# homopolymer/RAMBL

Measured on AMD Instinct MI355X. Metric: reads/sec into POA (150bp, ~1.5k-node graph), higher is better.
Workload: dtype f64

## Files before the change

rambl_amd/csrc/sc_api.cpp:

```cpp
#include <malloc.h>

#include <cmath>

#include "sc_ctx.hpp"

using namespace sc;
struct sc_ctx { Ctx c; sc_ctx(int device, const CtxPlan& plan) : c(device, plan) {} };

extern "C" {

int sc_host_plan(int stream_count, int local_world, double cpus, int* out) {
    if (!out || stream_count < 1) return SC_ERR_ARG;
    host_plan(stream_count, local_world > 0 ? local_world : local_world_size(), cpus > 0 ? cpus : cpu_budget_host(), out);
    return SC_OK;
}

int sc_ctx_create(int device, int stream_count, sc_ctx** out) {
    if (!out) return SC_ERR_ARG;
    *out = nullptr;
    setenv("GPU_MAX_HW_QUEUES", "16", 0);
    int ndev = 0;
    if (hipGetDeviceCount(&ndev) != hipSuccess || ndev <= 0 || device < 0 || device >= ndev) return SC_ERR_NO_DEVICE;
    hipDeviceProp_t prop;
    if (hipGetDeviceProperties(&prop, device) != hipSuccess) return SC_ERR_NO_DEVICE;
// ... 266 lines not shown
            f.labels[(size_t)e] = (uint8_t)(r >= 0 ? ent_sym[r] : 0);
        }
        for (int r = 0, q = 0; r < n_ent; r++) { f.ent_cn[(size_t)(e0 + r)] = ent_cn[r]; qoff[(size_t)(e0 + r)] = q; q += ent_cn[r]; }
        const hipStream_t st = w.st;
        const std::vector<int> mptr(mate_off, mate_off + n_reads + 1), midx(mate_idx, mate_idx + nm);
        JobDev jd = w.job_dev(w.passthrough, f, qoff, mptr, midx, n_reads, std::max<long>(Q, 1), n_ent, Q * n_sweeps);
        auto slot = [](int s) { return (s * 37 + 5) % MAXS; };
        std::vector<double> rows((size_t)jd.ll_stride * MAXS, 0.0);
        for (int s = 0; s < S; s++) std::memcpy(&rows[(size_t)slot(s) * jd.ll_stride], ll + (size_t)s * n_reads, sizeof(double) * n_reads);
        jd.ll = upload(w.passthrough, w.b_ll, rows, st);
        std::vector<uint8_t> hv(has, has + n_reads);
        hv.resize((size_t)n_reads + 8, 0);
        jd.has = upload(w.passthrough, w.b_has, hv, st);
        std::vector<double> u(U, U + Q * n_sweeps);
        u.resize((size_t)(Q * n_sweeps + 2048), 0.5);
        std::vector<float> uf(u.begin(), u.end());
        DevBuf b_u, b_uf;
        jd.U = upload(w.passthrough, b_u, u, st);
        jd.Uf = upload(w.passthrough, b_uf, uf, st);
        const JobDev* jd_dev = (const JobDev*)w.b_jobdev.ensure(sizeof(JobBlock));
        HIPCHK(hipMemcpyAsync((void*)jd_dev, &jd, sizeof jd, hipMemcpyHostToDevice, st));

        LevelParams& P = *w.Ph;
        for (int s = 0; s < S; s++) P.sp[s] = StrainParam{slot(s), E, 1, 0, a0[s], 0.0};
        LevelHdr H{};
        H.mode = MODE_SAMPLE; H.S = S; H.e0 = e0; H.e1 = E; H.Q = (int)Q; H.n_sweeps = n_sweeps;
        H.n_copy = 0; H.do_update = 0; H.seq = 1;
        std::memset(w.Rh, 0, sizeof(LevelResult));
        const LevelItem it = w.level_item(jd_dev, H, KMAX);
        const int kind = item_kind(it.kind);
        const int done = launch_level(st, it, n_reads);
        HIPCHK(hipGetLastError());
        HIPCHK(hipStreamSynchronize(st));
        const LevelResult& R = *w.Rh;
        if (R.seq != 1u || R.error) throw ScError(SC_ERR_INTERNAL, "the sampler level did not complete");
        for (int s = 0; s < S; s++) kdraw[s] = R.kdraw[s];
        std::memcpy(cnt, R.cnt, sizeof(unsigned) * (size_t)S * KMAX);
        out[0] = (long)R.n_draws; out[1] = (long)R.n_slow; out[2] = (long)R.n_exact; out[3] = (long)R.n_pass; out[4] = kind; out[5] = done;
        return SC_OK;
    } catch (const ScError& ex) { std::lock_guard<std::mutex> lk(ctx->mu); ctx->last_error = ex.what(); return ex.code; }
    catch (const std::exception& ex) { std::lock_guard<std::mutex> lk(ctx->mu); ctx->last_error = ex.what(); return SC_ERR_HIP; }
}
int sc_roi_release(sc_ctx* h, int handle) {
    if (!h) return SC_ERR_ARG;
    std::lock_guard<std::mutex> lk(h->c.mu);
    auto it = h->c.jobs.find(handle);
    if (it == h->c.jobs.end() || it->second->status != 1) return SC_ERR_ARG;
    h->c.jobs.erase(it);
    return SC_OK;
}

int sc_msa_align(sc_ctx* h, const char* seq_text, const int* seq_off, int n, char* rows_out, long cap, int* ncol_out) {
    if (!h || !seq_text || !seq_off || n < 1 || !ncol_out) return SC_ERR_ARG;
    Ctx* ctx = &h->c;
// ... 19 lines not shown
```

rambl_amd/csrc/sc_ctx.hpp:

```cpp
#pragma once
#include <atomic>
#include <condition_variable>
#include <deque>
#include <map>
#include <memory>
#include <mutex>
#include <thread>

#include "../../include/straincall_hip.h"
#include "sc_device.hpp"
#include "sc_fiber.hpp"
#include "sc_graph.hpp"
#include "sc_host.hpp"
#include "sc_plan.hpp"

namespace sc {

void launch_edge_support(hipStream_t st, const int* out_ptr, const int* out_node, const int* pool_ptr, const int* pool_rid,
                         const int* pool_cn, const uint8_t* node_is_end, const int* edge_src, int n_edges, int sorted,
                         int* support);
void launch_msa(hipStream_t st, const MsaDev& d);
void launch_thread(hipStream_t st, const ThreadDev& d, int* pool_sorted);
int init_graph_kernels();
bool level_wants_grid(int n_reads, const LevelHdr& h);
int launch_level_grid(hipStream_t st, const JobDev* job, int n_reads, const LevelHdr& h, int kind, const LevelParams* P, LevelResult* R, bool lone);
int launch_level(hipStream_t st, const LevelItem& it, int n_reads);
int level_kind(const LevelHdr& h);
int level_lds_kb(const LevelHdr& h, int K);
int level_table_capacity();
void launch_level_batch(hipStream_t st, int kind, const LevelBatch& b, int n);
void launch_level_any(hipStream_t st, const LevelBatch& b, int n);
void launch_resident(hipStream_t st, const ResidentArgs& a, int slots);
int init_level_kernels();
inline int init_kernels() { return init_level_kernels() | init_graph_kernels(); }

struct Job {
    int handle = 0;
    std::string ref;
    std::vector<AlignedRead> reads;
    std::vector<int> mate_off, mate_idx;
    sc_params params{};
    std::vector<std::string> seqs;
    std::vector<double> abund;
    std::string graph_dump, trace;
    std::vector<int> edge_support;
    std::vector<int> thr_count, thr_first, thr_pool;
    std::vector<int> thr_smin, thr_emin, thr_tmin;
    std::string thr_sym;
    sc_stats stats{};
// ... 118 lines not shown
};

struct Worker {
    Ctx* ctx = nullptr;
    ResidentGrid* grid = nullptr;
    Fiber* fib = nullptr;
    int slot = 0;
    hipStream_t st = nullptr;
    bool own_stream = false;
    hipEvent_t sync_ev = nullptr;
    std::atomic<int> level_state{0};
    std::string level_err;
    double t_seen = 0, wake_acc[2] = {0, 0};
    std::atomic<int> mslot{-1};
    std::atomic<double> t_posted{0};
    double t_batch_launched = 0;
    int batch_n = 0;
    int level_done = 0;
    hipEvent_t ev0 = nullptr, ev1 = nullptr;
    std::vector<hipEvent_t> ev_pool;
    size_t ev_used = 0;
    LevelParams* Ph = nullptr;
    LevelParams* Pm = nullptr;
    LevelParams* Pd = nullptr;
    LevelResult* Rh = nullptr;
    LevelResult* Rd = nullptr;
    bool own_blocks = false;
    unsigned seq = 0;
    DevBuf b_ent_rid, b_ent_cn, b_ent_lab_off, b_ent_lab_len, b_ent_first, b_ent_qoff, b_labels, b_mate_ptr, b_mate_idx,
        b_ll, b_has, b_isnew, b_tabA, b_tabLf, b_qcode, b_qent, b_quid, b_dlog, b_out_ptr, b_out_node, b_pool_ptr, b_pool_rid,
        b_pool_cn, b_isend, b_esrc, b_support, b_jobdev;
    DevBuf m_seqs, m_off, m_cols0, m_cols1, m_counts, m_moves, m_trace, m_out, m_edge;
    PinnedArena* stage = nullptr;
    PinnedArena passthrough;
    DevBuf t_ref, t_pos, t_seqoff, t_seq, t_cigoff, t_cigop, t_ciglen, t_lut, t_tabs, t_pool, t_pool2;
    FlatGraph flat;
    std::vector<int> ent_qoff_buf;
    bool setup_held = false;
    std::vector<ld> cnt_scratch;

    ~Worker();
    void init();
    void init_private(Ctx* c);
    void run();
    void process(Job& job);
    void complete_level(const LevelItem& it, int n_reads, bool timed);
    void wait_level();
    void finish_level(int state, const char* err = nullptr);
    void sync_stream();
    int msa_device(const std::vector<std::string>& seqs, std::vector<std::string>& rows);
    void thread_device(const std::string& G, const std::vector<AlignedRead>& R, const std::vector<std::vector<CigarOp>>& cig,
                       ThreadTables& T);
    JobDev job_dev(PinnedArena& ar, const FlatGraph& f, const std::vector<int>& ent_qoff, const std::vector<int>& mate_off,
// ... 19 lines not shown
```

rambl_amd/csrc/sc_device.hpp:

```cpp
#pragma once
#include <hip/hip_runtime.h>

#include <cstdint>
#include <type_traits>

namespace sc {

constexpr int MAXS = 128;
constexpr int KMAX = 16;
constexpr int KK = KMAX * KMAX;
constexpr int MAX_DRAWS = 40000;

enum LevelMode { MODE_HARD = 0, MODE_SAMPLE = 1 };

struct JobDev {
    const int* ent_rid;
    const int* ent_cn;
    const int* ent_lab_off;
    const int* ent_lab_len;
    const uint8_t* ent_first;
    const int* ent_qoff;
    const uint8_t* labels;
    const int* mate_ptr;
    const int* mate_idx;
    int n_reads;
    int K;
    int code_N;
    double* ll;
    long ll_stride;
    uint8_t* has;
    const double* U;
    const float* Uf;
    uint8_t* isnew;
    double* tabA;
    float* tabLf;
    uint8_t* qcode;
    int* qent;
    int* quid;
    long qcap;
    uint8_t* dlog;
    long dlog_cap;
};

struct JobBlock {
    JobDev job;
    unsigned long long t0;
};

struct LevelHdr {
    int mode;
    int S;
    int e0, e1;
    int has_dups;
    int any_multi;
    int Q;
    int n_sweeps;
    int n_copy;
    int do_update;
    int done;
    int copy_n;
    unsigned seq;
};
struct StrainParam {
    int slot;
    int lab_off, lab_len;
    int pad;
    double a0;
    double logpri;
};
struct LevelParams {
    int copy_src[MAXS], copy_dst[MAXS];
    StrainParam sp[MAXS];
    double lpt[MAXS * KK];
};

constexpr int N_SAMPLER_KINDS = 16;
__host__ __device__ constexpr int sampler_kind(int nb, bool rows_lds) { return 2 * nb - 1 + (rows_lds ? 1 : 0); }
__host__ __device__ constexpr bool kind_has_sampler(int kind) { return kind != 0; }
__host__ __device__ constexpr int kind_nb(int kind) { return (kind + 1) / 2; }
__host__ __device__ constexpr bool kind_rows_lds(int kind) { return kind % 2 == 0; }
__host__ __device__ constexpr int pack_kind(int kind, int lds_kb) { return kind | (lds_kb << 8); }
__host__ __device__ constexpr int item_kind(int word) { return word & 0xFF; }
__host__ __device__ constexpr int item_lds_kb(int word) { return (word >> 8) & 0xFFFF; }
static_assert(sampler_kind(1, false) == 1 && sampler_kind(8, true) == N_SAMPLER_KINDS && kind_nb(sampler_kind(5, true)) == 5 &&
              kind_rows_lds(sampler_kind(5, true)) && !kind_rows_lds(sampler_kind(5, false)) &&
              item_kind(pack_kind(13, 157)) == 13 && item_lds_kb(pack_kind(13, 157)) == 157, "level kind");
template <int NB = 1, class F>
__host__ __device__ __forceinline__ void with_sampler_variant(int kind, F&& f) {
    if constexpr (NB < 8) {
        if (kind_nb(kind) != NB) { with_sampler_variant<NB + 1>(kind, f); return; }
    }
    if (kind_rows_lds(kind)) f(std::integral_constant<int, NB>{}, std::true_type{});
    else f(std::integral_constant<int, NB>{}, std::false_type{});
}

struct LevelResult;
struct LevelItem {
// ... 82 lines not shown
```

rambl_amd/csrc/sc_level.hip:

```cpp
#include <hip/hip_runtime.h>
#include <math.h>
#include <stdint.h>
#include <stdlib.h>

#include <type_traits>

#include "sc_device.hpp"
#include "sc_sampler.hpp"

namespace sc {

constexpr int LDS_TOTAL = 160 * 1024 - 256;
constexpr int LDS_SMALL = 18 * 1024;
constexpr int LDS_BIG = LDS_TOTAL - LDS_SMALL;
static_assert(LDS_SMALL >= (int)(sizeof(double) * 2 * MAXS + sizeof(StrainParam) * MAXS + sizeof(unsigned) * MAXS * KMAX + sizeof(int) * 6 * MAXS + 64), "LDS_SMALL");
static_assert(LDS_BIG >= (int)(sizeof(double) * MAXS * 64), "LDS_BIG");

enum { LV_COPIES_DONE = 1, LV_ITEMS_DONE = 2, LV_HAS_DONE = 4, LV_HARD_DONE = 8, LV_SLOTS_DONE = 16, LV_ROWS_DONE = 32, LV_TICKED = 64 };
typedef const __attribute__((address_space(4))) JobDev KJob;

__device__ __forceinline__ void stage_params(const LevelHdr& h, const LevelParams* __restrict__ P, StrainParam* s_sp, int* s_copy,
                                             double* s_lpt, bool want_lpt, int K2, int tid, int nt) {
    const i4v* src_sp = reinterpret_cast<const i4v*>(P->sp);
    i4v* dst_sp = reinterpret_cast<i4v*>(s_sp);
// ... 120 lines not shown
        for (long idx = tid; idx < total; idx += nt) item((int)(idx / Rn), (int)(idx % Rn));
    } else {
        if (tid < S) for (int r = 0; r < Rn; r++) item(tid, r);
    }
    if (h.done & LV_HAS_DONE) { __syncthreads(); return; }
    __syncthreads();
    mark_present(job, h, tid, nt);
    __syncthreads();
}

template <bool BARRIER = true, class JD>
__device__ __forceinline__ void phase_slots(const JD& job, const LevelHdr& h, int tid, int nt) {
    const int e0 = h.e0, Rn = h.e1 - h.e0;
    for (int r = tid; r < Rn; r += nt) {
        const int e = e0 + r;
        const int rid = job.ent_rid[e], cn = job.ent_cn[e];
        const int qb = job.ent_qoff[e];
        const int mb = job.mate_ptr[rid], mn = job.mate_ptr[rid + 1] - mb;
        const uint8_t code = (job.ent_lab_len[e] == 1) ? job.labels[job.ent_lab_off[e]] : (uint8_t)0xFF;
        for (int i = 0; i < cn; i++) {
            const int k = cn - 1 - i;
            const int uid = (k < mn) ? job.mate_idx[mb + k] : -1;
            job.qent[qb + i] = r;
            job.quid[qb + i] = uid;
            job.qcode[qb + i] = code;
        }
    }
    if (BARRIER) __syncthreads();
}

__device__ __forceinline__ void finish_level(const LevelHdr& h, LevelResult* __restrict__ R, unsigned long long wall0, int tid) {
    __threadfence_system();
    __syncthreads();
    if (tid == 0) {
        R->level_wall = wall_clock64() - wall0;
        R->xcc = (int)(__builtin_amdgcn_s_getreg(20 | (3 << 11)) & 0xF);
        __hip_atomic_store(&R->seq, h.seq, __ATOMIC_RELEASE, __HIP_MEMORY_SCOPE_SYSTEM);
    }
}


template <class JD, class SL>
__device__ __forceinline__ void zero_unseen_mates(const JD& job, const LevelHdr& h, SL slot_of, int first, int step) {
    const long stride = job.ll_stride;
    for (int q = first; q < h.Q; q += step) {
        const int uid = job.quid[q];
// ... 9 lines not shown
        double* cell = col + (long)s * cs;
        *cell = exp(*cell - m) / norm;
    }
}

__device__ __forceinline__ void strain_sums(const double* prow, const uint8_t* qcode, int Q, int lane, double (&acc)[KMAX + 1]) {
#pragma unroll
    for (int b = 0; b <= KMAX; b++) acc[b] = 0.0;
    for (int q = lane; q < Q; q += 64) {
        const double p = prow[q];
        const int code = qcode[q];
        acc[KMAX] += p;
#pragma unroll
        for (int b = 0; b < KMAX; b++) acc[b] += (code == b) ? p : 0.0;
    }
#pragma unroll
    for (int b = 0; b <= KMAX; b++) {
        double v = acc[b];
        for (int off = 32; off > 0; off >>= 1) v += __shfl_down(v, off);
        acc[b] = v;
    }
}

template <int NB, class JD, class PUT>
__device__ __forceinline__ void weight_rows(const JD& job, const LevelHdr& h, const int* s_slot, PUT put4, int first, int step) {
    constexpr int SR = (NB <= 2) ? 16 * NB : 16;
    const int S = h.S, Q = h.Q, e0 = h.e0;
    const int stride = chain_w_stride(S);
    const long lstride = job.ll_stride;
    const float qnanf = __int_as_float(0x7fc00000);
    for (int q = first; q < Q; q += step) {
        const int rid = job.ent_rid[e0 + job.qent[q]], uid = job.quid[q];
        const bool hr = h.do_update ? true : job.has[rid] != 0;
        const bool hu = uid >= 0 && job.has[uid] != 0;
        const long Lf = (long)q * stride;
        auto cell = [&](int sx) __attribute__((always_inline)) -> double {
            const double* row = job.ll + (long)s_slot[sx] * lstride;
            double v = hr ? row[rid] : 0.0;
            if (hu) v += row[uid];
            return v;
        };
        double m = -INFINITY;
        double x[SR];
        if (NB <= 2) {
#pragma unroll
            for (int i = 0; i < SR; i++) { x[i] = -INFINITY; if (i < S) { x[i] = cell(i); m = fmax(m, x[i]); } }
        } else {
            for (int s0 = 0; s0 < S; s0 += SR) {
#pragma unroll
                for (int i = 0; i < SR; i++) if (s0 + i < S) m = fmax(m, cell(s0 + i));
            }
        }
        const bool flag = !(m >= -600.0);
        for (int s0 = 0; s0 < stride; s0 += SR) {
            if (NB > 2) {
#pragma unroll
                for (int i = 0; i < SR; i++) x[i] = (s0 + i < S) ? cell(s0 + i) : -INFINITY;
            }
#pragma unroll
            for (int i = 0; i < SR; i += 4) {
                if (s0 + i < stride) {
                    f4v w;
#pragma unroll
                    for (int k = 0; k < 4; k++) {
                        const int sx = s0 + i + k;
                        const float wk = sx < S ? (flag ? qnanf : exp_weight(x[i + k] - m)) : 0.0f;
                        if (k == 0) w.x = wk; else if (k == 1) w.y = wk; else if (k == 2) w.z = wk; else w.w = wk;
                    }
                    put4(Lf + s0 + i, w);
                }
            }
        }
        if (q == Q - 1) for (int i = 0; i < 16; i += 4) put4(Lf + stride + i, f4v{0.0f, 0.0f, 0.0f, 0.0f});
    }
}

struct LevelLds {
    double* s_a; double* s_p; unsigned* s_cnt; int* s_slot; unsigned* s_kf; float* s_a0f; int* s_x; int* s_copy; int* s_lab;
    StrainParam* s_sp; unsigned char* s_big;
};
__device__ __forceinline__ LevelLds level_lds(unsigned char* raw) {
    LevelLds l;
    l.s_a = reinterpret_cast<double*>(raw);
    l.s_p = l.s_a + MAXS;
    l.s_sp = reinterpret_cast<StrainParam*>(l.s_p + MAXS);
    l.s_cnt = reinterpret_cast<unsigned*>(l.s_sp + MAXS);
    l.s_slot = reinterpret_cast<int*>(l.s_cnt + MAXS * KMAX);
    l.s_kf = reinterpret_cast<unsigned*>(l.s_slot + MAXS);
    l.s_a0f = reinterpret_cast<float*>(l.s_kf + MAXS);
    l.s_copy = reinterpret_cast<int*>(l.s_a0f + MAXS);
    l.s_lab = l.s_copy + 2 * MAXS;
    l.s_x = l.s_lab + MAXS;
    l.s_big = raw + LDS_SMALL;
    return l;
}

// ... 244 lines not shown
#pragma unroll
                for (int i = 0; i < 5; i++) dst[i] = src[i];
                last = s_item.h.seq;
                served++;
                const long ip = s_item.P - a.P_base, ir = s_item.R - a.R_base;
                if (ip < 0 || ip >= a.n_blocks || ir != ip || a.P_base + ip != s_item.P || s_item.job == nullptr) cmd = 2;
            }
            s_cmd = cmd;
        }
        __syncthreads();
        if (s_cmd != 1) break;
        level_dispatch(&s_item);
        __syncthreads();
    }
    if (tid == 0) {
        __hip_atomic_store(&mb->levels, served, __ATOMIC_RELAXED, __HIP_MEMORY_SCOPE_SYSTEM);
        __hip_atomic_store(&mb->state, s_cmd == 2 ? 3u : 2u, __ATOMIC_RELEASE, __HIP_MEMORY_SCOPE_SYSTEM);
    }
}
__device__ __forceinline__ void grid_tick(unsigned long long* t0) {
    if (t0 && blockIdx.x == 0 && blockIdx.y == 0 && threadIdx.x == 0) *t0 = wall_clock64();
}

__global__ __launch_bounds__(256) void k_level_copy(const JobDev* jp, LevelHdr h, const LevelParams* __restrict__ P, unsigned long long* t0) {
    grid_tick(t0);
    KJob& job = *(KJob*)jp;
    const int c = blockIdx.y;
    const double2* src = reinterpret_cast<const double2*>(job.ll + (long)P->copy_src[c] * job.ll_stride);
    double2* dst = reinterpret_cast<double2*>(job.ll + (long)P->copy_dst[c] * job.ll_stride);
    const int n2 = ((h.copy_n < job.n_reads ? h.copy_n : job.n_reads) + 1) >> 1;
    for (int i = blockIdx.x * blockDim.x + threadIdx.x; i < n2; i += gridDim.x * blockDim.x) dst[i] = src[i];
}

__global__ __launch_bounds__(256) void k_level_update(const JobDev* jp, LevelHdr h, const LevelParams* __restrict__ P, unsigned long long* t0) {
    __shared__ double s_row[MAXS * KMAX];
    __shared__ double s_diag[MAXS * KMAX];
    __shared__ int s_slot[MAXS], s_lab[MAXS];
    grid_tick(t0);
    KJob& job = *(KJob*)jp;
    const int tid = threadIdx.x, nt = blockDim.x;
    const int S = h.S, K = job.K, e0 = h.e0, Rn = h.e1 - h.e0, codeN = job.code_N;
    const long total = (long)S * Rn;
    const long per = ((total + gridDim.x - 1) / gridDim.x + nt - 1) / nt * nt;
    const long lo = (long)blockIdx.x * per, hi = lo + per < total ? lo + per : total;
    if (lo >= hi) return;
    const int sa = (int)(lo / Rn), sb = (int)((hi - 1) / Rn);
    for (int s = sa + tid; s <= sb; s += nt) { s_slot[s] = P->sp[s].slot; s_lab[s] = job.labels[P->sp[s].lab_off]; }
    __syncthreads();
    for (int i = sa * KMAX + tid; i < (sb + 1) * KMAX; i += nt) {
        const int sx = i / KMAX, b = i % KMAX, a = s_lab[sx];
        const double* lp = P->lpt + (long)sx * K * K;
        s_row[i] = (a < K && b < K) ? lp[a * K + b] : 0.0;
        s_diag[i] = (b < K) ? lp[b * K + b] : 0.0;
    }
    __syncthreads();
    const long stride = job.ll_stride;
    for (long idx = lo + tid; idx < hi; idx += nt) {
        const int sx = (int)(idx / Rn), e = e0 + (int)(idx % Rn);
        const int rid = job.ent_rid[e];
        const int b = job.labels[job.ent_lab_off[e]];
        const bool fresh = job.ent_first[e] && !job.has[rid];
        if (sx == 0) job.isnew[e - e0] = fresh ? 1 : 0;
        int a = s_lab[sx];
        const bool wild = (a == codeN);
        if (wild) a = b;
        const double val = (a < K && b < K) ? (wild ? s_diag[sx * KMAX + b] : s_row[sx * KMAX + b]) : __longlong_as_double(0x7ff8000000000000ll);
        double* cell = job.ll + (long)s_slot[sx] * stride + rid;
        *cell = fresh ? val : (*cell + val);
    }
}

__global__ __launch_bounds__(256) void k_level_entries(const JobDev* jp, LevelHdr h, int has, int slots, unsigned long long* t0) {
    grid_tick(t0);
    KJob& job = *(KJob*)jp;
    const int first = blockIdx.x * blockDim.x + threadIdx.x, step = gridDim.x * blockDim.x;
    if (has) mark_present(job, h, first, step);
    if (slots) phase_slots<false>(job, h, first, step);
}

template <int NB>
__global__ __launch_bounds__(64) void k_level_rows(const JobDev* jp, LevelHdr h, const LevelParams* __restrict__ P, unsigned long long* t0) {
    __shared__ int s_slot[MAXS];
    grid_tick(t0);
    KJob& job = *(KJob*)jp;
    for (int s = threadIdx.x; s < h.S; s += blockDim.x) s_slot[s] = P->sp[s].slot;
    __syncthreads();
    SC_GLOBAL float* rows_g = (SC_GLOBAL float*)job.tabLf;
    weight_rows<NB>(job, h, s_slot, [&](long idx, f4v v) __attribute__((always_inline)) { *(SC_GLOBAL f4v*)(rows_g + idx) = v; },
                    blockIdx.x * blockDim.x + threadIdx.x, gridDim.x * blockDim.x);
}

__global__ __launch_bounds__(256) void k_hard_mates(const JobDev* jp, LevelHdr h, const LevelParams* __restrict__ P) {
    __shared__ int s_slot[MAXS];
    KJob& job = *(KJob*)jp;
    for (int s = threadIdx.x; s < h.S; s += blockDim.x) s_slot[s] = P->sp[s].slot;
    __syncthreads();
    zero_unseen_mates(job, h, [&](int s) { return s_slot[s]; }, blockIdx.x * blockDim.x + threadIdx.x, gridDim.x * blockDim.x);
}
__global__ __launch_bounds__(256) void k_hard_resp(const JobDev* jp, LevelHdr h, const LevelParams* __restrict__ P) {
    __shared__ int s_slot[MAXS];
    __shared__ double s_logpri[MAXS];
    KJob& job = *(KJob*)jp;
    const int S = h.S, e0 = h.e0;
    for (int s = threadIdx.x; s < S; s += blockDim.x) { s_slot[s] = P->sp[s].slot; s_logpri[s] = P->sp[s].logpri; }
    __syncthreads();
    const long stride = job.ll_stride;
    for (int q = blockIdx.x * blockDim.x + threadIdx.x; q < h.Q; q += gridDim.x * blockDim.x) {
        const int rid = job.ent_rid[e0 + job.qent[q]], uid = job.quid[q];
        if (uid >= 0) job.has[uid] = 1;
        double* col = job.tabA + q;
        double m = -INFINITY;
        for (int s = 0; s < S; s++) {
// ... 38 lines not shown
constexpr long GRID_COPY_WORDS = 1L << 19;
constexpr long GRID_HARD = 1L << 18;
constexpr long WIDE_ITEMS = 1L << 12;
static long grid_min(long dflt) {
    static const long forced = [] { const char* e = getenv("SC_GRID_MIN"); return e ? atol(e) : -1L; }();
    return forced >= 0 ? forced : dflt;
}
static long wide_min() {
    static const long forced = [] { const char* e = getenv("SC_WIDE_MIN"); return e ? atol(e) : -1L; }();
    return forced >= 0 ? forced : WIDE_ITEMS;
}
static bool hard_on_grid(const LevelHdr& h) {
    return h.mode == MODE_HARD && h.do_update && (long)h.S * (h.e1 - h.e0) > grid_min(GRID_ITEMS) && !h.has_dups && !h.any_multi &&
           (long)h.S * h.Q > grid_min(GRID_HARD) && h.e1 > h.e0;
}
bool level_wants_grid(int n_reads, const LevelHdr& h) {
    const long items = (long)h.S * (h.e1 - h.e0);
    return (h.do_update && items > grid_min(GRID_ITEMS) && !h.has_dups && !h.any_multi) || (long)h.n_copy * n_reads > grid_min(GRID_COPY_WORDS);
}
static int grid_blocks(long n, int per, int most) {
    const long g = (n + per - 1) / per;
    return (int)(g < 1 ? 1 : (g > most ? most : g));
}
int launch_level_grid(hipStream_t st, const JobDev* job, int n_reads, const LevelHdr& h, int kind, const LevelParams* P, LevelResult* R, bool lone) {
    const int S = h.S, Rn = h.e1 - h.e0;
    const long items = (long)S * Rn;
    const bool upd = h.do_update && Rn > 0;
    const bool wide = lone && items > wide_min() && Rn > 0 && S > 0;
    const bool update_on_grid = upd && !h.has_dups && !h.any_multi && (items > grid_min(GRID_ITEMS) || wide);
    const bool rows_on_grid = wide && kind_has_sampler(kind) && h.Q > 0 && (update_on_grid || !upd);
    const bool hard = update_on_grid && hard_on_grid(h);
    int done = 0;
    unsigned long long* t0 = lone ? &reinterpret_cast<JobBlock*>(const_cast<JobDev*>(job))->t0 : nullptr;
    if (h.n_copy > 0 && ((long)h.n_copy * n_reads > grid_min(GRID_COPY_WORDS) || update_on_grid || rows_on_grid)) {
        const int n = h.copy_n < n_reads ? h.copy_n : n_reads;
        hipLaunchKernelGGL(k_level_copy, dim3(grid_blocks((n + 1) >> 1, 1024, 256), h.n_copy), dim3(256), 0, st, job, h, P, t0);
        t0 = nullptr;
        done |= LV_COPIES_DONE;
    }
    if (update_on_grid) {
        hipLaunchKernelGGL(k_level_update, dim3(grid_blocks(items, 512, 1024)), dim3(256), 0, st, job, h, P, t0);
        t0 = nullptr;
        done |= LV_ITEMS_DONE | LV_HAS_DONE;
    }
    const bool slots = rows_on_grid || hard;
    if (update_on_grid || slots) {
        hipLaunchKernelGGL(k_level_entries, dim3(grid_blocks(Rn, 256, 1024)), dim3(256), 0, st, job, h, update_on_grid ? 1 : 0, slots ? 1 : 0, t0);
        t0 = nullptr;
        if (slots) done |= LV_SLOTS_DONE;
    }
    if (rows_on_grid) {
        with_sampler_variant(kind, [&](auto nb, auto) {
            hipLaunchKernelGGL((k_level_rows<decltype(nb)::value>), dim3(grid_blocks(h.Q, 64, 128)), dim3(64), 0, st, job, h, P, t0);
        });
        done |= LV_ROWS_DONE;
    }
    if (hard) {
        const int gq = grid_blocks(h.Q, 256, 2048);
        hipLaunchKernelGGL(k_hard_mates, dim3(gq), dim3(256), 0, st, job, h, P);
        hipLaunchKernelGGL(k_hard_resp, dim3(gq), dim3(256), 0, st, job, h, P);
        hipLaunchKernelGGL(k_hard_sums, dim3(S), dim3(64), 0, st, job, h, P, R);
        done |= LV_HARD_DONE;
    }
    return done ? (done | (lone ? LV_TICKED : 0)) : 0;
}
int level_kind(const LevelHdr& h) {
    const int S = h.S, Q = h.Q, Rn = h.e1 - h.e0;
    const bool chain = h.mode == MODE_SAMPLE && h.n_sweeps > 0 && S > 1 && Rn > 0;
    if (!chain) return 0;
    const bool wl = ((long)Q * chain_w_stride(S) + 16) * 4 <= (long)CHAINW_ROWS_BYTES;
    int nb = (S + 15) / 16;
    nb = nb < 1 ? 1 : (nb > 8 ? 8 : nb);
    return sampler_kind(nb, wl);
}
int level_lds_kb(const LevelHdr& h, int K) {
    const int kind = level_kind(h);
// ... 9 lines not shown
    if (need > LDS_TOTAL) need = LDS_TOTAL;
    return (int)((need + 1023) / 1024);
}
static size_t batch_lds(const LevelBatch& b, int n) {
    int kb = 0;
    for (int i = 0; i < n; i++) { const int k = item_lds_kb(b.it[i].kind); kb = k > kb ? k : kb; }
    size_t bytes = (size_t)kb * 1024;
    if (kb == 0 || bytes > (size_t)LDS_TOTAL) bytes = LDS_TOTAL;
    return bytes;
}
void launch_level_any(hipStream_t st, const LevelBatch& b, int n) {
    hipLaunchKernelGGL(k_level_any, dim3(n), dim3(CHAIN_THREADS), batch_lds(b, n), st, b);
}
void launch_level_batch(hipStream_t st, int kind, const LevelBatch& b, int n) {
    const size_t lds = batch_lds(b, n);
    if (!kind_has_sampler(kind)) {
        hipLaunchKernelGGL(k_level, dim3(n), dim3(512), lds, st, b);
        return;
    }
    with_sampler_variant(kind, [&](auto nb, auto rows_lds) {
        hipLaunchKernelGGL((k_level_sample<decltype(nb)::value, decltype(rows_lds)::value>), dim3(n), dim3(CHAIN_THREADS), lds, st, b);
    });
}
int launch_level(hipStream_t st, const LevelItem& it, int n_reads) {
    LevelBatch batch;
    batch.it[0] = it;
    LevelItem& b = batch.it[0];
    b.h.done |= launch_level_grid(st, b.job, n_reads, b.h, item_kind(b.kind), b.P, b.R, true);
    launch_level_batch(st, item_kind(b.kind), batch, 1);
    return b.h.done;
}
void launch_resident(hipStream_t st, const ResidentArgs& a, int slots) {
    hipLaunchKernelGGL(k_level_resident, dim3(slots), dim3(CHAIN_THREADS), LDS_TOTAL, st, a);
}
}
#ifdef SC_CHAIN_PROF
extern "C" int sc_debug_chain_prof(unsigned long long* out) {
    return (int)hipMemcpyFromSymbol(out, HIP_SYMBOL(sc::g_chain_prof), sizeof(unsigned long long) * 12);
}
#endif
```

rambl_amd/csrc/sc_region.cpp:

```cpp
#include "sc_ctx.hpp"

namespace sc {

int Worker::msa_device(const std::vector<std::string>& seqs, std::vector<std::string>& rows) {
    const int n = (int)seqs.size();
    std::vector<int> off(n + 1, 0);
    std::string packed;
    for (int i = 0; i < n; i++) { packed += seqs[i]; off[i + 1] = (int)packed.size(); }
    const int cmax = (int)packed.size() + 1;
    size_t longest = 0;
    for (int i = 1; i < n; i++) longest = std::max(longest, seqs[i].size());
    MsaDev d;
    char* dseq = (char*)m_seqs.ensure(packed.size() + 1);
    int* doff = (int*)m_off.ensure(sizeof(int) * (n + 1));
    stage->h2d(dseq, packed.data(), packed.size(), st);
    stage->h2d(doff, off.data(), sizeof(int) * (n + 1), st);
    d.seqs = dseq; d.seq_off = doff; d.n = n; d.cmax = cmax;
    d.cols[0] = (char*)m_cols0.ensure((size_t)cmax * n);
    d.cols[1] = (char*)m_cols1.ensure((size_t)cmax * n);
    d.counts = (int*)m_counts.ensure(sizeof(int) * 11 * (size_t)cmax);
    d.mv_stride = (int)((longest + 1 + 63) / 64) * 64;
    d.moves = (uint8_t*)m_moves.ensure((size_t)(cmax + 1) * (size_t)d.mv_stride);
    d.edge = (int*)m_edge.ensure(sizeof(int) * 2 * (size_t)(cmax + 1));
    d.trace = (int*)m_trace.ensure(sizeof(int) * 2 * (size_t)(cmax + 64));
// ... 110 lines not shown
}

JobDev Worker::job_dev(PinnedArena& ar, const FlatGraph& f, const std::vector<int>& ent_qoff, const std::vector<int>& mate_off,
                       const std::vector<int>& mate_idx, int n_reads, long qcap, int max_entries, long max_draws) {
    JobDev jd{};
    jd.ent_rid = upload(ar, b_ent_rid, f.ent_rid, st);
    jd.ent_cn = upload(ar, b_ent_cn, f.ent_cn, st);
    jd.ent_lab_off = upload(ar, b_ent_lab_off, f.ent_lab_off, st);
    jd.ent_lab_len = upload(ar, b_ent_lab_len, f.ent_lab_len, st);
    jd.ent_first = upload(ar, b_ent_first, f.ent_first, st);
    jd.ent_qoff = upload(ar, b_ent_qoff, ent_qoff, st);
    jd.labels = upload(ar, b_labels, f.labels, st);
    jd.mate_ptr = upload(ar, b_mate_ptr, mate_off, st);
    jd.mate_idx = upload(ar, b_mate_idx, mate_idx, st);
    jd.n_reads = n_reads; jd.K = f.K; jd.code_N = f.code_N;
    jd.ll_stride = ((long)n_reads + 3) & ~3L;
    jd.isnew = (uint8_t*)b_isnew.ensure((size_t)max_entries + 8);
    jd.qcap = qcap;
    jd.tabA = (double*)b_tabA.ensure(sizeof(double) * (size_t)qcap * MAXS);
    jd.tabLf = (float*)b_tabLf.ensure(sizeof(float) * (size_t)(std::min<long>(qcap, MAX_DRAWS) + 4) * 136);
    jd.qcode = (uint8_t*)b_qcode.ensure((size_t)qcap + 8);
    jd.qent = (int*)b_qent.ensure(sizeof(int) * (size_t)qcap);
    jd.quid = (int*)b_quid.ensure(sizeof(int) * (size_t)qcap);
    jd.dlog_cap = std::max<long>(max_draws, 1);
    jd.dlog = (uint8_t*)b_dlog.ensure((size_t)jd.dlog_cap + 8);
    return jd;
}

void Worker::cluster(Job& job, const PoGraph& g, FlatGraph& f) {
    const int n_reads = (int)job.reads.size();
    const double t_cluster0 = now_ms();

    const int final_e0 = (int)f.ent_rid.size();
    long total_copies = 0;
    {
        int qo = 0;
        for (int i = 0; i < n_reads; i++) {
            f.ent_rid.push_back(i); f.ent_cn.push_back(job.reads[i].cn); f.ent_lab_off.push_back(0);
            f.ent_lab_len.push_back(0); f.ent_first.push_back(1);
            qo += job.reads[i].cn;
        }
        total_copies = qo;
    }
    std::vector<int>& ent_qoff = ent_qoff_buf;
    ent_qoff.assign(f.ent_rid.size(), 0);
    int max_level_entries = n_reads, max_level_q = 0;
// ... 114 lines not shown
```

rambl_amd/csrc/sc_sched.cpp:

```cpp
#include "sc_ctx.hpp"

namespace sc {

PinnedArena* ArenaPool::lease(PinnedArena* passthrough) {
    if (limit <= 0) { passthrough->on = false; return passthrough; }
    for (;;) {
        {
            std::lock_guard<std::mutex> lk(mu);
            if (!free_arenas.empty()) { PinnedArena* a = free_arenas.back(); free_arenas.pop_back(); a->reset(); return a; }
            if ((int)arenas.size() < limit) { arenas.emplace_back(new PinnedArena()); return arenas.back().get(); }
        }
        if (FiberPool::in_fiber()) FiberPool::yield(); else std::this_thread::yield();
    }
}
void ArenaPool::release(PinnedArena* a) {
    std::lock_guard<std::mutex> lk(mu);
    free_arenas.push_back(a);
}
void SetupGate::enter(Worker* w) {
    {
        std::lock_guard<std::mutex> lk(mu);
        if (setups < limit) { setups++; return; }
        waiters.push_back(w);
    }
// ... 323 lines not shown
        Mailbox& mb = grid->mail.p[m];
        mb.item = it;
        __atomic_store_n(&mb.seq, want, __ATOMIC_RELEASE);
        const double t = now_ms();
        t_posted.store(t, std::memory_order_release);
        t_batch_launched = t; batch_n = 1;
        if (alone) {
            for (unsigned spins = 0; __atomic_load_n(&Rh->seq, __ATOMIC_ACQUIRE) != want;) {
                __builtin_ia32_pause();
                if (++spins % (1u << 20) == 0)
                    if (const char* why = resident_failure(mb, &Rh->seq, want, t)) throw HipError(why);
            }
        } else {
            level_state.store(1, std::memory_order_release);
            grid->watch->arm((size_t)slot, want);
            ctx->pool->ensure_poller();
            wait_level();
        }
        __atomic_store_n(&grid->mail_done[(size_t)m], want, __ATOMIC_RELEASE);
    } else if (alone) {
        hipStream_t ls = ctx->launch->st;
        if (timed) HIPCHK(hipEventRecord(ev0, ls));
        (void)hipGetLastError();
        level_done = launch_level(ls, it, n_reads);
        { const hipError_t le = hipGetLastError(); if (le != hipSuccess) throw HipError(std::string("level kernel launch: ") + hipGetErrorString(le)); }
        if (timed) HIPCHK(hipEventRecord(ev1, ls));
        t_batch_launched = now_ms(); batch_n = 1;
        (void)hipStreamQuery(ls);
        for (unsigned spins = 0; __atomic_load_n(&Rh->seq, __ATOMIC_ACQUIRE) != want;) {
            __builtin_ia32_pause();
            if ((++spins & 0x3FFFFu) == 0) {
                const hipError_t e = hipStreamQuery(ls);
                if (e == hipSuccess) { if (__atomic_load_n(&Rh->seq, __ATOMIC_ACQUIRE) != want) throw HipError("a level kernel ended without its completion stamp"); }
                else if (e != hipErrorNotReady) throw HipError(std::string("level kernel: ") + hipGetErrorString(e));
            }
        }
    } else {
        t_posted.store(now_ms(), std::memory_order_release);
        ctx->server->submit(LevelRequest{this, it, item_kind(it.kind), timed});
        wait_level();
    }
}

void Worker::run() {
    for (;;) {
        std::shared_ptr<Job> job;
        bool parked = false;
// ... 125 lines not shown
```

rambl_amd/csrc/sc_walk.cpp:

```cpp
#include <cmath>

#include "sc_ctx.hpp"

namespace sc {

struct Model {
    int ks = KMAX;
    ld sub[KK];
    ld comp[6]; ld Z;
    ld lsub[KK];
    double lpc[KK];
    uint16_t stale[KMAX];
    unsigned dirty;
    Model() = default;
    Model(const Model& o) { *this = o; }
    Model& operator=(const Model& o) {
        ks = o.ks; Z = o.Z; dirty = o.dirty;
        const size_t n = (size_t)ks * ks;
        std::memcpy(sub, o.sub, sizeof(ld) * n); std::memcpy(lsub, o.lsub, sizeof(ld) * n); std::memcpy(lpc, o.lpc, sizeof(double) * n);
        std::memcpy(comp, o.comp, sizeof comp); std::memcpy(stale, o.stale, sizeof stale);
        return *this;
    }
};
struct HStrain {
// ... 173 lines not shown
                            level_strains[merged[j]].abundance += level_strains[i].abundance;
                            break;
                        }
                    if (j == merged.size()) merged.push_back(i);
                }
                std::vector<HStrain> kept;
                std::vector<char> keep(level_strains.size(), 0);
                for (int j : merged) { kept.push_back(level_strains[j]); keep[j] = 1; }
                for (size_t i = 0; i < level_strains.size(); i++) if (!keep[i]) drop(level_strains[i]);
                level_strains.swap(kept);
                final_strains = level_strains;
            }
        }
    }
    void run_level(int mode, int e0, int e1, int Q, int n_sweeps, bool do_update, const std::vector<HStrain>& sv,
                              bool has_dups, bool any_multi) {
        LevelParams& P = *w.Ph;
        const int S = (int)sv.size();
        LevelHdr H{};
        H.mode = mode; H.S = S; H.e0 = e0; H.e1 = e1; H.has_dups = has_dups; H.any_multi = any_multi; H.Q = Q;
        H.n_sweeps = n_sweeps; H.do_update = do_update ? 1 : 0;
        H.n_copy = (int)pending_copies.size();
        H.copy_n = do_update ? level_hi[(size_t)cur_level] : n_reads;
        for (int c = 0; c < H.n_copy; c++) { P.copy_src[c] = pending_copies[c].first; P.copy_dst[c] = pending_copies[c].second; }
        pending_copies.clear();
        {
            uint64_t seen[2] = {0, 0};
            for (int s = 0; s < S; s++) {
                const int r = sv[s].slot;
                if (r < 0 || r >= MAXS || (seen[r >> 6] >> (r & 63)) & 1) throw ScError(SC_ERR_INTERNAL, "two candidates share a read_loglik row");
                seen[r >> 6] |= 1ull << (r & 63);
            }
        }
        for (int s = 0; s < S; s++) {
            const int nd = sv[s].node;
            if (nd >= 0) { __builtin_prefetch(&f.node_lab_off[(size_t)nd]); __builtin_prefetch(&f.node_lab_len[(size_t)nd]); }
            if (do_update) {
                const Model& hm = models[(size_t)sv[s].model];
                __builtin_prefetch(&hm.dirty); __builtin_prefetch(&hm.stale[0]);
                for (int o = 0; o < K * K; o += 8) __builtin_prefetch(&hm.lpc[o]);
            }
        }
        ld za = 0;
        for (int s = 0; s < S; s++) za += sv[s].abundance;
        for (int s = 0; s < S; s++) {
            StrainParam& sp = P.sp[s];
            sp.slot = sv[s].slot;
            sp.lab_off = sv[s].node >= 0 ? f.node_lab_off[sv[s].node] : 0;
            sp.lab_len = sv[s].node >= 0 ? f.node_lab_len[sv[s].node] : 0;
            la_cache[s] = (sp.lab_len == 1) ? (int)f.labels[(size_t)sp.lab_off] : -1;
            sp.pad = 0;
            sp.a0 = (double)sv[s].abundance;
            sp.logpri = (mode == MODE_HARD) ? (double)logl(sv[s].abundance / za) : 0.0;
            if (!do_update) continue;
            Model& hm = models[(size_t)sv[s].model];
            for (int a = 0; a < K; a++) {
                if (!(hm.dirty & (1u << a))) continue;
                const ld lc = logl(a < 6 ? hm.comp[a] : (ld)0);
                for (int b = 0; b < K; b++) {
                    if (hm.stale[a] & (1u << b)) hm.lsub[a * K + b] = logl(hm.sub[a * K + b]);
                    hm.lpc[a * K + b] = (double)(hm.lsub[a * K + b] - lc);
                }
                hm.stale[a] = 0;
            }
            hm.dirty = 0;
            double* dst = P.lpt + (size_t)s * K * K;
            std::memcpy(dst, hm.lpc, sizeof(double) * (size_t)K * K);
        }
        const bool chain = (mode == MODE_SAMPLE) && S > 1 && n_sweeps > 0;
        if (mode == MODE_SAMPLE && (long)n_sweeps * Q > jd.dlog_cap) throw ScError(SC_ERR_INTERNAL, "a level draws more than the region's draw log holds");
        const bool timed = chain && pa.want_timing && !w.grid;
        const bool lone = !w.grid && w.ctx->workers.size() == 1;
        if (!lone && level_wants_grid(jd.n_reads, H)) {
            const size_t bytes = offsetof(LevelParams, lpt) + sizeof(double) * (size_t)S * K * K;
            HIPCHK(hipMemcpyAsync(w.Pd, w.Ph, bytes, hipMemcpyHostToDevice, w.st));
            H.done = launch_level_grid(w.st, jd_dev, jd.n_reads, H, level_kind(H), w.Pd, w.Rd, false);
            w.sync_stream();
        }
        const int ms = w.mslot.load(std::memory_order_relaxed);
        H.seq = ms >= 0 ? ++w.grid->mail_seq[(size_t)ms] : ++w.seq;
        if (timed) {
            if (w.ev_used + 2 > w.ev_pool.size()) {
                hipEvent_t a = nullptr, b = nullptr;
                HIPCHK(hipEventCreate(&a)); HIPCHK(hipEventCreate(&b));
                w.ev_pool.push_back(a); w.ev_pool.push_back(b);
            }
            w.ev0 = w.ev_pool[w.ev_used]; w.ev1 = w.ev_pool[w.ev_used + 1];
            w.ev_used += 2;
        }
        const double t_launched = level_log ? now_ms() : 0.0;
        lap(0);
        const LevelItem it = w.level_item(jd_dev, H, K);
        w.complete_level(it, jd.n_reads, timed);
        t_mark = now_ms();
        sc_stats& stats = job.stats;
        stats.level_launches++;
        if (chain) {
            stats.sampler_launches++; stats.sampler_read_copies += Q;
            stats.draws += (long)Rh->n_draws; stats.exact_draws += (long)Rh->n_exact; stats.slow_draws += (long)Rh->n_slow;
// ... 277 lines not shown
```

Before: 15140.

## Pass slot/label params by value and split row-weight work across 8-lane groups

Slot indices, labels and copy rows are packed into a small GridParams struct passed as kernel arguments, so the copy, update and rows kernels no longer read them from the device LevelParams buffer. k_level_rows now gives each query to a group of 8 lanes, with a shuffle reduction for the row max, instead of one thread per query. A new qrid array saves the ent_rid indirection. The cost is larger kernel argument blocks, an extra per-query store, and more grid blocks.

```diff
diff --git a/rambl_amd/csrc/sc_api.cpp b/rambl_amd/csrc/sc_api.cpp
--- a/rambl_amd/csrc/sc_api.cpp
+++ b/rambl_amd/csrc/sc_api.cpp
@@ -312,14 +312,18 @@
         HIPCHK(hipMemcpyAsync((void*)jd_dev, &jd, sizeof jd, hipMemcpyHostToDevice, st));
 
         LevelParams& P = *w.Ph;
-        for (int s = 0; s < S; s++) P.sp[s] = StrainParam{slot(s), E, 1, 0, a0[s], 0.0};
+        for (int s = 0; s < S; s++) {
+            P.sp[s] = StrainParam{slot(s), E, 1, 0, a0[s], 0.0};
+            w.gp.slot[s] = (uint8_t)slot(s);
+            w.gp.lab[s] = f.labels[(size_t)E];
+        }
         LevelHdr H{};
         H.mode = MODE_SAMPLE; H.S = S; H.e0 = e0; H.e1 = E; H.Q = (int)Q; H.n_sweeps = n_sweeps;
         H.n_copy = 0; H.do_update = 0; H.seq = 1;
         std::memset(w.Rh, 0, sizeof(LevelResult));
         const LevelItem it = w.level_item(jd_dev, H, KMAX);
         const int kind = item_kind(it.kind);
-        const int done = launch_level(st, it, n_reads);
+        const int done = launch_level(st, it, w.gp, n_reads);
         HIPCHK(hipGetLastError());
         HIPCHK(hipStreamSynchronize(st));
         const LevelResult& R = *w.Rh;
diff --git a/rambl_amd/csrc/sc_ctx.hpp b/rambl_amd/csrc/sc_ctx.hpp
--- a/rambl_amd/csrc/sc_ctx.hpp
+++ b/rambl_amd/csrc/sc_ctx.hpp
@@ -23,8 +23,8 @@
 void launch_thread(hipStream_t st, const ThreadDev& d, int* pool_sorted);
 int init_graph_kernels();
 bool level_wants_grid(int n_reads, const LevelHdr& h);
-int launch_level_grid(hipStream_t st, const JobDev* job, int n_reads, const LevelHdr& h, int kind, const LevelParams* P, LevelResult* R, bool lone);
-int launch_level(hipStream_t st, const LevelItem& it, int n_reads);
+int launch_level_grid(hipStream_t st, const JobDev* job, int n_reads, const LevelHdr& h, int kind, const GridParams& g, const LevelParams* P, LevelResult* R, bool lone);
+int launch_level(hipStream_t st, const LevelItem& it, const GridParams& g, int n_reads);
 int level_kind(const LevelHdr& h);
 int level_lds_kb(const LevelHdr& h, int K);
 int level_table_capacity();
@@ -189,13 +189,14 @@
     size_t ev_used = 0;
     LevelParams* Ph = nullptr;
     LevelParams* Pm = nullptr;
+    GridParams gp{};
     LevelParams* Pd = nullptr;
     LevelResult* Rh = nullptr;
     LevelResult* Rd = nullptr;
     bool own_blocks = false;
     unsigned seq = 0;
     DevBuf b_ent_rid, b_ent_cn, b_ent_lab_off, b_ent_lab_len, b_ent_first, b_ent_qoff, b_labels, b_mate_ptr, b_mate_idx,
-        b_ll, b_has, b_isnew, b_tabA, b_tabLf, b_qcode, b_qent, b_quid, b_dlog, b_out_ptr, b_out_node, b_pool_ptr, b_pool_rid,
+        b_ll, b_has, b_isnew, b_tabA, b_tabLf, b_qcode, b_qent, b_quid, b_qrid, b_dlog, b_out_ptr, b_out_node, b_pool_ptr, b_pool_rid,
         b_pool_cn, b_isend, b_esrc, b_support, b_jobdev;
     DevBuf m_seqs, m_off, m_cols0, m_cols1, m_counts, m_moves, m_trace, m_out, m_edge;
     PinnedArena* stage = nullptr;
diff --git a/rambl_amd/csrc/sc_device.hpp b/rambl_amd/csrc/sc_device.hpp
--- a/rambl_amd/csrc/sc_device.hpp
+++ b/rambl_amd/csrc/sc_device.hpp
@@ -1,6 +1,7 @@
 #pragma once
 #include <hip/hip_runtime.h>
 
+#include <cstddef>
 #include <cstdint>
 #include <type_traits>
 
@@ -40,7 +41,11 @@
     long qcap;
     uint8_t* dlog;
     long dlog_cap;
+    int* qrid;
 };
+static_assert(offsetof(JobDev, quid) == 168 && offsetof(JobDev, qcap) == 176 && offsetof(JobDev, dlog) == 184 &&
+              offsetof(JobDev, dlog_cap) == 192 && offsetof(JobDev, qrid) == 200 && sizeof(JobDev) == 208,
+              "the fields the urn chain reads keep their offsets; new fields go last");
 
 struct JobBlock {
     JobDev job;
@@ -73,6 +78,14 @@
     StrainParam sp[MAXS];
     double lpt[MAXS * KK];
 };
+
+struct GridParams {
+    uint8_t slot[MAXS];
+    uint8_t lab[MAXS];
+    uint8_t copy_src[MAXS], copy_dst[MAXS];
+};
+static_assert(MAXS - 1 <= UINT8_MAX && KMAX <= UINT8_MAX, "a row index and a symbol code fit GridParams' bytes");
+static_assert(sizeof(GridParams) == 4 * MAXS, "GridParams is packed");
 
 constexpr int N_SAMPLER_KINDS = 16;
 __host__ __device__ constexpr int sampler_kind(int nb, bool rows_lds) { return 2 * nb - 1 + (rows_lds ? 1 : 0); }
diff --git a/rambl_amd/csrc/sc_level.hip b/rambl_amd/csrc/sc_level.hip
--- a/rambl_amd/csrc/sc_level.hip
+++ b/rambl_amd/csrc/sc_level.hip
@@ -166,6 +166,7 @@
             const int k = cn - 1 - i;
             const int uid = (k < mn) ? job.mate_idx[mb + k] : -1;
             job.qent[qb + i] = r;
+            job.qrid[qb + i] = rid;
             job.quid[qb + i] = uid;
             job.qcode[qb + i] = code;
         }
@@ -221,24 +222,46 @@
     }
 }
 
+struct SlotCells {
+    const double* ll; long lstride; int rid, uid; bool hr, hu;
+    __device__ __forceinline__ double operator()(int row) const {
+        const double* r = ll + (long)row * lstride;
+        double v = hr ? r[rid] : 0.0;
+        if (hu) v += r[uid];
+        return v;
+    }
+};
+template <class JD>
+__device__ __forceinline__ SlotCells slot_cells(const JD& job, const LevelHdr& h, int rid, int uid) {
+    const bool hr = h.do_update ? true : job.has[rid] != 0;
+    const bool hu = uid >= 0 && job.has[uid] != 0;
+    return SlotCells{job.ll, job.ll_stride, rid, uid, hr, hu};
+}
+__device__ __forceinline__ bool row_flagged(double m) { return !(m >= -600.0); }
+__device__ __forceinline__ f4v row_block(const double* x, int s0, int S, double m, bool flag) {
+    const float qnanf = __int_as_float(0x7fc00000);
+    f4v w;
+#pragma unroll
+    for (int k = 0; k < 4; k++) {
+        const float wk = s0 + k < S ? (flag ? qnanf : exp_weight(x[k] - m)) : 0.0f;
+        if (k == 0) w.x = wk; else if (k == 1) w.y = wk; else if (k == 2) w.z = wk; else w.w = wk;
+    }
+    return w;
+}
+template <class PUT>
+__device__ __forceinline__ void row_tail(PUT put4, long end, int first, int step) {
+    for (int i = first; i < 4; i += step) put4(end + 4 * i, f4v{0.0f, 0.0f, 0.0f, 0.0f});
+}
+
 template <int NB, class JD, class PUT>
 __device__ __forceinline__ void weight_rows(const JD& job, const LevelHdr& h, const int* s_slot, PUT put4, int first, int step) {
     constexpr int SR = (NB <= 2) ? 16 * NB : 16;
     const int S = h.S, Q = h.Q, e0 = h.e0;
     const int stride = chain_w_stride(S);
-    const long lstride = job.ll_stride;
-    const float qnanf = __int_as_float(0x7fc00000);
     for (int q = first; q < Q; q += step) {
-        const int rid = job.ent_rid[e0 + job.qent[q]], uid = job.quid[q];
-        const bool hr = h.do_update ? true : job.has[rid] != 0;
-        const bool hu = uid >= 0 && job.has[uid] != 0;
+        const SlotCells cells = slot_cells(job, h, job.ent_rid[e0 + job.qent[q]], job.quid[q]);
         const long Lf = (long)q * stride;
-        auto cell = [&](int sx) __attribute__((always_inline)) -> double {
-            const double* row = job.ll + (long)s_slot[sx] * lstride;
-            double v = hr ? row[rid] : 0.0;
-            if (hu) v += row[uid];
-            return v;
-        };
+        auto cell = [&](int sx) __attribute__((always_inline)) -> double { return cells(s_slot[sx]); };
         double m = -INFINITY;
         double x[SR];
         if (NB <= 2) {
@@ -250,27 +273,17 @@
                 for (int i = 0; i < SR; i++) if (s0 + i < S) m = fmax(m, cell(s0 + i));
             }
         }
-        const bool flag = !(m >= -600.0);
+        const bool flag = row_flagged(m);
         for (int s0 = 0; s0 < stride; s0 += SR) {
             if (NB > 2) {
 #pragma unroll
                 for (int i = 0; i < SR; i++) x[i] = (s0 + i < S) ? cell(s0 + i) : -INFINITY;
             }
 #pragma unroll
-            for (int i = 0; i < SR; i += 4) {
-                if (s0 + i < stride) {
-                    f4v w;
-#pragma unroll
-                    for (int k = 0; k < 4; k++) {
-                        const int sx = s0 + i + k;
-                        const float wk = sx < S ? (flag ? qnanf : exp_weight(x[i + k] - m)) : 0.0f;
-                        if (k == 0) w.x = wk; else if (k == 1) w.y = wk; else if (k == 2) w.z = wk; else w.w = wk;
-                    }
-                    put4(Lf + s0 + i, w);
-                }
-            }
-        }
-        if (q == Q - 1) for (int i = 0; i < 16; i += 4) put4(Lf + stride + i, f4v{0.0f, 0.0f, 0.0f, 0.0f});
+            for (int i = 0; i < SR; i += 4)
+                if (s0 + i < stride) put4(Lf + s0 + i, row_block(x + i, s0 + i, S, m, flag));
+        }
+        if (q == Q - 1) row_tail(put4, Lf + stride, 0, 1);
     }
 }
 
@@ -561,17 +574,17 @@
     if (t0 && blockIdx.x == 0 && blockIdx.y == 0 && threadIdx.x == 0) *t0 = wall_clock64();
 }
 
-__global__ __launch_bounds__(256) void k_level_copy(const JobDev* jp, LevelHdr h, const LevelParams* __restrict__ P, unsigned long long* t0) {
+__global__ __launch_bounds__(256) void k_level_copy(const JobDev* jp, LevelHdr h, GridParams g, unsigned long long* t0) {
     grid_tick(t0);
     KJob& job = *(KJob*)jp;
     const int c = blockIdx.y;
-    const double2* src = reinterpret_cast<const double2*>(job.ll + (long)P->copy_src[c] * job.ll_stride);
-    double2* dst = reinterpret_cast<double2*>(job.ll + (long)P->copy_dst[c] * job.ll_stride);
+    const double2* src = reinterpret_cast<const double2*>(job.ll + (long)g.copy_src[c] * job.ll_stride);
+    double2* dst = reinterpret_cast<double2*>(job.ll + (long)g.copy_dst[c] * job.ll_stride);
     const int n2 = ((h.copy_n < job.n_reads ? h.copy_n : job.n_reads) + 1) >> 1;
     for (int i = blockIdx.x * blockDim.x + threadIdx.x; i < n2; i += gridDim.x * blockDim.x) dst[i] = src[i];
 }
 
-__global__ __launch_bounds__(256) void k_level_update(const JobDev* jp, LevelHdr h, const LevelParams* __restrict__ P, unsigned long long* t0) {
+__global__ __launch_bounds__(256) void k_level_update(const JobDev* jp, LevelHdr h, GridParams g, const LevelParams* __restrict__ P, unsigned long long* t0) {
     __shared__ double s_row[MAXS * KMAX];
     __shared__ double s_diag[MAXS * KMAX];
     __shared__ int s_slot[MAXS], s_lab[MAXS];
@@ -584,7 +597,7 @@
     const long lo = (long)blockIdx.x * per, hi = lo + per < total ? lo + per : total;
     if (lo >= hi) return;
     const int sa = (int)(lo / Rn), sb = (int)((hi - 1) / Rn);
-    for (int s = sa + tid; s <= sb; s += nt) { s_slot[s] = P->sp[s].slot; s_lab[s] = job.labels[P->sp[s].lab_off]; }
+    for (int s = sa + tid; s <= sb; s += nt) { s_slot[s] = g.slot[s]; s_lab[s] = g.lab[s]; }
     __syncthreads();
     for (int i = sa * KMAX + tid; i < (sb + 1) * KMAX; i += nt) {
         const int sx = i / KMAX, b = i % KMAX, a = s_lab[sx];
@@ -617,16 +630,48 @@
     if (slots) phase_slots<false>(job, h, first, step);
 }
 
+constexpr int ROWS_G = 8;
 template <int NB>
-__global__ __launch_bounds__(64) void k_level_rows(const JobDev* jp, LevelHdr h, const LevelParams* __restrict__ P, unsigned long long* t0) {
-    __shared__ int s_slot[MAXS];
+__global__ __launch_bounds__(64) void k_level_rows(const JobDev* jp, LevelHdr h, GridParams g, unsigned long long* t0) {
+    constexpr int NBLK = (4 * NB + 1 + ROWS_G - 1) / ROWS_G;
+    static_assert(64 % ROWS_G == 0 && ROWS_G <= 8, "a group lies inside a wavefront");
     grid_tick(t0);
     KJob& job = *(KJob*)jp;
-    for (int s = threadIdx.x; s < h.S; s += blockDim.x) s_slot[s] = P->sp[s].slot;
-    __syncthreads();
+    const int S = h.S, Q = h.Q;
+    const int stride = chain_w_stride(S), nblk = stride >> 2;
+    const int k = threadIdx.x % ROWS_G;
     SC_GLOBAL float* rows_g = (SC_GLOBAL float*)job.tabLf;
-    weight_rows<NB>(job, h, s_slot, [&](long idx, f4v v) __attribute__((always_inline)) { *(SC_GLOBAL f4v*)(rows_g + idx) = v; },
-                    blockIdx.x * blockDim.x + threadIdx.x, gridDim.x * blockDim.x);
+    auto put4 = [&](long idx, f4v v) __attribute__((always_inline)) { *(SC_GLOBAL f4v*)(rows_g + idx) = v; };
+    const int per_wave = 64 / ROWS_G;
+    for (int q0 = blockIdx.x * per_wave; q0 < Q; q0 += gridDim.x * per_wave) {
+        const int q = q0 + threadIdx.x / ROWS_G;
+        const bool live = q < Q;
+        double x[NBLK][4];
+        double m = -INFINITY;
+        if (live) {
+            const SlotCells cells = slot_cells(job, h, job.qrid[q], job.quid[q]);
+#pragma unroll
+            for (int j = 0; j < NBLK; j++) {
+#pragma unroll
+                for (int i = 0; i < 4; i++) {
+                    const int sx = 4 * (k + ROWS_G * j) + i;
+                    x[j][i] = -INFINITY;
+                    if (sx < S) { x[j][i] = cells(g.slot[sx]); m = fmax(m, x[j][i]); }
+                }
+            }
+        }
+#pragma unroll
+        for (int o = 1; o < ROWS_G; o <<= 1) m = fmax(m, __shfl_xor(m, o));
+        if (!live) continue;
+        const bool flag = row_flagged(m);
+        const long Lf = (long)q * stride;
+#pragma unroll
+        for (int j = 0; j < NBLK; j++) {
+            const int blk = k + ROWS_G * j;
+            if (blk < nblk) put4(Lf + 4 * blk, row_block(x[j], 4 * blk, S, m, flag));
+        }
+        if (q == Q - 1) row_tail(put4, Lf + stride, k, ROWS_G);
+    }
 }
 
 __global__ __launch_bounds__(256) void k_hard_mates(const JobDev* jp, LevelHdr h, const LevelParams* __restrict__ P) {
@@ -711,7 +756,9 @@
     const long g = (n + per - 1) / per;
     return (int)(g < 1 ? 1 : (g > most ? most : g));
 }
-int launch_level_grid(hipStream_t st, const JobDev* job, int n_reads, const LevelHdr& h, int kind, const LevelParams* P, LevelResult* R, bool lone) {
+struct GridUpdateArgs { const JobDev* job; LevelHdr h; GridParams g; const LevelParams* P; unsigned long long* t0; };
+static_assert(sizeof(GridUpdateArgs) + 256 <= 4096, "kernel-argument segment of the grid kernels");
+int launch_level_grid(hipStream_t st, const JobDev* job, int n_reads, const LevelHdr& h, int kind, const GridParams& g, const LevelParams* P, LevelResult* R, bool lone) {
     const int S = h.S, Rn = h.e1 - h.e0;
     const long items = (long)S * Rn;
     const bool upd = h.do_update && Rn > 0;
@@ -723,12 +770,12 @@
     unsigned long long* t0 = lone ? &reinterpret_cast<JobBlock*>(const_cast<JobDev*>(job))->t0 : nullptr;
     if (h.n_copy > 0 && ((long)h.n_copy * n_reads > grid_min(GRID_COPY_WORDS) || update_on_grid || rows_on_grid)) {
         const int n = h.copy_n < n_reads ? h.copy_n : n_reads;
-        hipLaunchKernelGGL(k_level_copy, dim3(grid_blocks((n + 1) >> 1, 1024, 256), h.n_copy), dim3(256), 0, st, job, h, P, t0);
+        hipLaunchKernelGGL(k_level_copy, dim3(grid_blocks((n + 1) >> 1, 1024, 256), h.n_copy), dim3(256), 0, st, job, h, g, t0);
         t0 = nullptr;
         done |= LV_COPIES_DONE;
     }
     if (update_on_grid) {
-        hipLaunchKernelGGL(k_level_update, dim3(grid_blocks(items, 512, 1024)), dim3(256), 0, st, job, h, P, t0);
+        hipLaunchKernelGGL(k_level_update, dim3(grid_blocks(items, 512, 1024)), dim3(256), 0, st, job, h, g, P, t0);
         t0 = nullptr;
         done |= LV_ITEMS_DONE | LV_HAS_DONE;
     }
@@ -740,7 +787,7 @@
     }
     if (rows_on_grid) {
         with_sampler_variant(kind, [&](auto nb, auto) {
-            hipLaunchKernelGGL((k_level_rows<decltype(nb)::value>), dim3(grid_blocks(h.Q, 64, 128)), dim3(64), 0, st, job, h, P, t0);
+            hipLaunchKernelGGL((k_level_rows<decltype(nb)::value>), dim3(grid_blocks(h.Q, 64 / ROWS_G, 4096)), dim3(64), 0, st, job, h, g, t0);
         });
         done |= LV_ROWS_DONE;
     }
@@ -796,11 +843,11 @@
         hipLaunchKernelGGL((k_level_sample<decltype(nb)::value, decltype(rows_lds)::value>), dim3(n), dim3(CHAIN_THREADS), lds, st, b);
     });
 }
-int launch_level(hipStream_t st, const LevelItem& it, int n_reads) {
+int launch_level(hipStream_t st, const LevelItem& it, const GridParams& g, int n_reads) {
     LevelBatch batch;
     batch.it[0] = it;
     LevelItem& b = batch.it[0];
-    b.h.done |= launch_level_grid(st, b.job, n_reads, b.h, item_kind(b.kind), b.P, b.R, true);
+    b.h.done |= launch_level_grid(st, b.job, n_reads, b.h, item_kind(b.kind), g, b.P, b.R, true);
     launch_level_batch(st, item_kind(b.kind), batch, 1);
     return b.h.done;
 }
diff --git a/rambl_amd/csrc/sc_region.cpp b/rambl_amd/csrc/sc_region.cpp
--- a/rambl_amd/csrc/sc_region.cpp
+++ b/rambl_amd/csrc/sc_region.cpp
@@ -156,6 +156,7 @@
     jd.qcode = (uint8_t*)b_qcode.ensure((size_t)qcap + 8);
     jd.qent = (int*)b_qent.ensure(sizeof(int) * (size_t)qcap);
     jd.quid = (int*)b_quid.ensure(sizeof(int) * (size_t)qcap);
+    jd.qrid = (int*)b_qrid.ensure(sizeof(int) * (size_t)qcap);
     jd.dlog_cap = std::max<long>(max_draws, 1);
     jd.dlog = (uint8_t*)b_dlog.ensure((size_t)jd.dlog_cap + 8);
     return jd;
diff --git a/rambl_amd/csrc/sc_sched.cpp b/rambl_amd/csrc/sc_sched.cpp
--- a/rambl_amd/csrc/sc_sched.cpp
+++ b/rambl_amd/csrc/sc_sched.cpp
@@ -369,7 +369,7 @@
         hipStream_t ls = ctx->launch->st;
         if (timed) HIPCHK(hipEventRecord(ev0, ls));
         (void)hipGetLastError();
-        level_done = launch_level(ls, it, n_reads);
+        level_done = launch_level(ls, it, gp, n_reads);
         { const hipError_t le = hipGetLastError(); if (le != hipSuccess) throw HipError(std::string("level kernel launch: ") + hipGetErrorString(le)); }
         if (timed) HIPCHK(hipEventRecord(ev1, ls));
         t_batch_launched = now_ms(); batch_n = 1;
diff --git a/rambl_amd/csrc/sc_walk.cpp b/rambl_amd/csrc/sc_walk.cpp
--- a/rambl_amd/csrc/sc_walk.cpp
+++ b/rambl_amd/csrc/sc_walk.cpp
@@ -219,7 +219,13 @@
         H.n_sweeps = n_sweeps; H.do_update = do_update ? 1 : 0;
         H.n_copy = (int)pending_copies.size();
         H.copy_n = do_update ? level_hi[(size_t)cur_level] : n_reads;
-        for (int c = 0; c < H.n_copy; c++) { P.copy_src[c] = pending_copies[c].first; P.copy_dst[c] = pending_copies[c].second; }
+        GridParams& G = w.gp;
+        for (int c = 0; c < H.n_copy; c++) {
+            P.copy_src[c] = pending_copies[c].first; P.copy_dst[c] = pending_copies[c].second;
+            if ((unsigned)P.copy_src[c] >= (unsigned)MAXS || (unsigned)P.copy_dst[c] >= (unsigned)MAXS)
+                throw ScError(SC_ERR_INTERNAL, "a row copy names a row outside the read_loglik matrix");
+            G.copy_src[c] = (uint8_t)P.copy_src[c]; G.copy_dst[c] = (uint8_t)P.copy_dst[c];
+        }
         pending_copies.clear();
         {
             uint64_t seen[2] = {0, 0};
@@ -247,6 +253,8 @@
             sp.lab_len = sv[s].node >= 0 ? f.node_lab_len[sv[s].node] : 0;
             la_cache[s] = (sp.lab_len == 1) ? (int)f.labels[(size_t)sp.lab_off] : -1;
             sp.pad = 0;
+            G.slot[s] = (uint8_t)sp.slot;
+            G.lab[s] = sp.lab_len >= 1 ? f.labels[(size_t)sp.lab_off] : (uint8_t)0;
             sp.a0 = (double)sv[s].abundance;
             sp.logpri = (mode == MODE_HARD) ? (double)logl(sv[s].abundance / za) : 0.0;
             if (!do_update) continue;
@@ -271,7 +279,7 @@
         if (!lone && level_wants_grid(jd.n_reads, H)) {
             const size_t bytes = offsetof(LevelParams, lpt) + sizeof(double) * (size_t)S * K * K;
             HIPCHK(hipMemcpyAsync(w.Pd, w.Ph, bytes, hipMemcpyHostToDevice, w.st));
-            H.done = launch_level_grid(w.st, jd_dev, jd.n_reads, H, level_kind(H), w.Pd, w.Rd, false);
+            H.done = launch_level_grid(w.st, jd_dev, jd.n_reads, H, level_kind(H), w.gp, w.Pd, w.Rd, false);
             w.sync_stream();
         }
         const int ms = w.mslot.load(std::memory_order_relaxed);
```

Measured after the change: 15510, median of 6. 1.02x the previous value.
